# Kaixhin/Rainbow

Hardware: NVIDIA B200
Metric: learner updates/sec (batch32, 1M buffer, 51 atoms) (higher is better)
Workload: dtype f32

## Files before the change

### include/rainbow_b200.h

```cpp
#ifndef RAINBOW_B200_H
#define RAINBOW_B200_H

#include <stdint.h>

#ifdef __cplusplus
extern "C" {
#endif

#define RB_ABI_VERSION 2

#define RB_OK 0
#define RB_ERR_INVAL (-22)
#define RB_ERR_RANGE (-34)
#define RB_ERR_CUDA (-5)

#define RB_FRAME_BYTES 7056
#define RB_MAX_WINDOW 64
#define RB_MAX_ATOMS 128
#define RB_MAX_NOISY_LAYERS 8
#define RB_MAX_PEERS 8
#define RB_APPEND_BATCH 8


typedef void* rb_stream_t;

enum {
  RB_K_TREE_UPDATE = 0, RB_K_TREE_FIND, RB_K_TREE_SAMPLE, RB_K_GATHER, RB_K_ITER_STATES, RB_K_APPEND, RB_K_C51,
  RB_K_NOISY_RESAMPLE, RB_K_NOISY_COMPOSE, RB_K_SQNORM, RB_K_CLIP_ADAM, RB_K_HEAD_FC1, RB_K_HEAD_FC2, RB_K_HEAD_LOGITS,
  RB_K_HEAD_WGRAD2, RB_K_HEAD_DH, RB_K_HEAD_BWD1, RB_K_NOISE_FACTORS, RB_K_C51_DUELING, RB_K_BIAS_GRAD, RB_K_Q_VALUES,
  RB_K_HEAD_REDUCE1, RB_K_CONV_WGRAD, RB_KERNEL_COUNT
};

int rb_abi_version(void);
const char* rb_last_error(void);

int rb_profile_enable(int on);
int rb_profile_collect(int kernel_id, double* total_ms, int* launches);

int rb_tree_update(float* tree, int64_t tree_start, int64_t size, const int64_t* tree_idx,
                   const float* raw_priority, float omega, int omega_is_applied, int B, float* running_max,
                   int32_t* status, const int32_t* gate, rb_stream_t stream);

int rb_tree_find(const float* tree, int64_t tree_start, int64_t size, const double* values, int B, float* probs,
                 int64_t* data_idx, int64_t* tree_idx, rb_stream_t stream);

int rb_tree_sample(const float* tree, int64_t tree_start, int64_t size, const int64_t* ring_state, int n,
                   int history, const double* u01, int u01_attempts, uint64_t seed, uint64_t* rng_counter, int B,
                   float beta, const float* beta_dev, int max_attempts, float* probs, int64_t* data_idx,
                   int64_t* tree_idx, float* weights, int32_t* status, rb_stream_t stream);

int rb_gather(const uint8_t* frames, const int32_t* timestep, const int32_t* action, const float* reward,
              const uint8_t* nonterminal, int64_t size, const int64_t* data_idx, int B, int history, int n,
              const float* gamma_pow, float* states, float* next_states, int64_t* actions, float* returns,
              float* nonterminals, rb_stream_t stream);

int rb_iter_states(const uint8_t* frames, const int32_t* timestep, int64_t size, int64_t first, int count,
                   int history, float* out, rb_stream_t stream);

int rb_append(float* tree, int64_t tree_start, int64_t size, uint8_t* frames, int32_t* timestep, int32_t* action,
              float* reward, uint8_t* nonterminal, int64_t* ring_state, float* running_max,
              const float* state_last_frame, int32_t action_value, float reward_value, int terminal,
              rb_stream_t stream);

int rb_append_batch(float* tree, int64_t tree_start, int64_t size, uint8_t* frames, int32_t* timestep, int32_t* action,
                    float* reward, uint8_t* nonterminal, int64_t* ring_state, float* running_max,
                    const float* const* last_frames, const int32_t* actions, const float* rewards, const int32_t* terminals,
                    int k, rb_stream_t stream);

int rb_c51_loss_grad(const float* q_online_s, const float* q_online_ns, const float* q_target_ns,
                     const int64_t* actions, const float* returns, const float* nonterminals,
                     const float* weights, const float* support, float vmin, float vmax, float delta_z,
                     float gamma_n, int B, int A, int Z, float* loss, float* grad_q_online_s, float* m_out,
                     int64_t* astar_out, rb_stream_t stream);

int rb_noisy_resample(float* const* weight_eps, float* const* bias_eps, const int* in_features,
                      const int* out_features, int n_layers, const float* x_in, const float* x_out, uint64_t seed,
                      uint64_t* rng_counter, rb_stream_t stream);

int rb_noisy_outer(float* const* weight_eps, float* const* bias_eps, const int* in_features, const int* out_features,
                   int n_layers, const float* f_in, const float* f_out, rb_stream_t stream);

int rb_noise_factors(float* f_in, int n_in, float* f_out, int n_out, const float* x_in, const float* x_out, uint64_t seed,
                     uint64_t* rng_counter, rb_stream_t stream);

typedef struct rb_head_params {
  const float* w1_mu[2];    const float* w1_sigma[2];
  const float* b1_mu[2];    const float* b1_sigma[2];
  const float* w2_mu[2];    const float* w2_sigma[2];
  const float* b2_mu[2];    const float* b2_sigma[2];
  const float* eps_in1[2];  const float* eps_out1[2];
  const float* eps_in2[2];  const float* eps_out2[2];
  int conv_features, hidden, atoms, actions;
} rb_head_params;

typedef struct rb_head_grads {
  float* w1_mu[2]; float* w1_sigma[2]; float* b1_mu[2]; float* b1_sigma[2];
  float* w2_mu[2]; float* w2_sigma[2]; float* b2_mu[2]; float* b2_sigma[2];
} rb_head_grads;

int rb_head_splits(int conv_features, int hidden, int* s1, int* s2);
int rb_head_ticket_count(void);
int rb_head_debug(int flags);

int rb_head_forward(const rb_head_params* p, const float* x_lo, int m_lo, const float* x_hi, int m_hi, float* part1, float* part2,
                    int32_t* tickets, float* h, float* z, rb_stream_t stream);

int rb_head_logits(const float* z, int M, int actions, int atoms, float* q, rb_stream_t stream);

#define RB_HEAD_BWD_WGRAD2 1
#define RB_HEAD_BWD_DH 2
#define RB_HEAD_BWD_LAYER1 4
#define RB_HEAD_BWD_ALL 7
int rb_head_backward(const rb_head_params* p, const rb_head_grads* g, const float* x, const float* h, const float* dz, int B,
                     float* dh_scratch, float* dx, int relu_mask_x, int parts, rb_stream_t stream);

int rb_q_values(const float* z, int M, int actions, int atoms, const float* support, float* q, int64_t* best_action,
                float* best_q, rb_stream_t stream);

int rb_bias_grad(const float* grad_out, int B, int C, int HW, float* out, rb_stream_t stream);

int rb_conv_wgrad_scratch_elems(int B, int IC, int IH, int OC, int K, int stride);
int rb_conv_wgrad(const float* grad_out, const float* input, int B, int IC, int IH, int IW, int OC, int K, int stride,
                  float* partials, float* out, float* bias_out, rb_stream_t stream);

int rb_c51_dueling_loss_grad(const float* z_online, const float* z_target, int actions_n, int atoms, const int64_t* actions,
                             const float* returns, const float* nonterminals, const float* weights, const float* support,
                             float vmin, float vmax, float delta_z, float gamma_n, int B, float* loss, float* dz, float* m_out,
                             int64_t* astar_out, rb_stream_t stream);

int rb_noisy_compose(const float* mu, const float* sigma, const float* eps, int64_t count, float* out,
                     rb_stream_t stream);

int rb_clip_adam_scratch_elems(void);
int rb_clip_adam(float* param, const float* grad, float* exp_avg, float* exp_avg_sq, int64_t P, float grad_scale,
                 float max_norm, float lr, float beta1, float beta2, float eps, int64_t* step_count,
                 double* partial_sums, float* norm_out, const int32_t* gate, rb_stream_t stream);

int rb_peer_scratch_bytes(void);
int rb_peer_reduce(const float* const* peer_grad, uint64_t* const* peer_flags, int world, int rank, int seg, int64_t seg_begin,
                   int64_t seg_len, float grad_scale, float* gred_part, const uint64_t* epoch, void* scratch,
                   rb_stream_t stream);
int rb_peer_adam_gather(float* const* peer_param, uint64_t* const* peer_flags, double* const* peer_norms, int world, int rank,
                        int n_seg, const int64_t* seg_begin, const int64_t* seg_len, const float* gred, float* exp_avg,
                        float* exp_avg_sq, float max_norm, float lr, float beta1, float beta2, float eps, int64_t* step_count,
                        uint64_t* epoch, void* scratch, float* norm_out, float* multicast_param, rb_stream_t stream);
int rb_peer_clip_adam(const float* const* peer_grad, float* const* peer_param, uint64_t* const* peer_flags,
                      double* const* peer_norms, int world, int rank, int64_t P, float* gred, float* exp_avg,
                      float* exp_avg_sq, float grad_scale, float max_norm, float lr, float beta1, float beta2, float eps,
                      int64_t* step_count, uint64_t* epoch, void* scratch, float* norm_out, rb_stream_t stream);

#ifdef __cplusplus
}
#endif
#endif
```

### rainbow_b200/_lib.py

```python
import ctypes as C
import os

from . import _build

_lib = None

_vp, _i64, _i32, _f32, _u64 = C.c_void_p, C.c_int64, C.c_int, C.c_float, C.c_uint64

class HeadParams(C.Structure):
    _fields_ = [(n, _vp * 2) for n in ("w1_mu", "w1_sigma", "b1_mu", "b1_sigma", "w2_mu", "w2_sigma", "b2_mu", "b2_sigma",
                                        "eps_in1", "eps_out1", "eps_in2", "eps_out2")] + \
               [(n, C.c_int) for n in ("conv_features", "hidden", "atoms", "actions")]


class HeadGrads(C.Structure):
    _fields_ = [(n, _vp * 2) for n in ("w1_mu", "w1_sigma", "b1_mu", "b1_sigma", "w2_mu", "w2_sigma", "b2_mu", "b2_sigma")]


_hp, _hg = C.POINTER(HeadParams), C.POINTER(HeadGrads)

SIGNATURES = {
    "rb_abi_version": (C.c_int, []),
    "rb_last_error": (C.c_char_p, []),
    "rb_profile_enable": (C.c_int, [_i32]),
    "rb_profile_collect": (C.c_int, [_i32, C.POINTER(C.c_double), C.POINTER(C.c_int)]),
    "rb_tree_update": (C.c_int, [_vp, _i64, _i64, _vp, _vp, _f32, _i32, _i32, _vp, _vp, _vp, _vp]),
    "rb_tree_find": (C.c_int, [_vp, _i64, _i64, _vp, _i32, _vp, _vp, _vp, _vp]),
    "rb_tree_sample": (C.c_int, [_vp, _i64, _i64, _vp, _i32, _i32, _vp, _i32, _u64, _vp, _i32, _f32, _vp, _i32,
                                 _vp, _vp, _vp, _vp, _vp, _vp]),
    "rb_gather": (C.c_int, [_vp, _vp, _vp, _vp, _vp, _i64, _vp, _i32, _i32, _i32, _vp, _vp, _vp, _vp, _vp, _vp, _vp]),
    "rb_iter_states": (C.c_int, [_vp, _vp, _i64, _i64, _i32, _i32, _vp, _vp]),
    "rb_append": (C.c_int, [_vp, _i64, _i64, _vp, _vp, _vp, _vp, _vp, _vp, _vp, _vp, C.c_int32, _f32, _i32, _vp]),
    "rb_append_batch": (C.c_int, [_vp, _i64, _i64, _vp, _vp, _vp, _vp, _vp, _vp, _vp, _vp, _vp, _vp, _vp, _i32, _vp]),
    "rb_c51_loss_grad": (C.c_int, [_vp, _vp, _vp, _vp, _vp, _vp, _vp, _vp, _f32, _f32, _f32, _f32, _i32, _i32, _i32,
                                   _vp, _vp, _vp, _vp, _vp]),
    "rb_noisy_resample": (C.c_int, [_vp, _vp, _vp, _vp, _i32, _vp, _vp, _u64, _vp, _vp]),
    "rb_noisy_outer": (C.c_int, [_vp, _vp, _vp, _vp, _i32, _vp, _vp, _vp]),
    "rb_noise_factors": (C.c_int, [_vp, _i32, _vp, _i32, _vp, _vp, _u64, _vp, _vp]),
    "rb_head_splits": (C.c_int, [_i32, _i32, C.POINTER(C.c_int), C.POINTER(C.c_int)]),
    "rb_head_ticket_count": (C.c_int, []),
    "rb_head_debug": (C.c_int, [_i32]),
    "rb_head_forward": (C.c_int, [_hp, _vp, _i32, _vp, _i32, _vp, _vp, _vp, _vp, _vp, _vp]),
    "rb_head_logits": (C.c_int, [_vp, _i32, _i32, _i32, _vp, _vp]),
    "rb_head_backward": (C.c_int, [_hp, _hg, _vp, _vp, _vp, _i32, _vp, _vp, _i32, _i32, _vp]),
    "rb_bias_grad": (C.c_int, [_vp, _i32, _i32, _i32, _vp, _vp]),
    "rb_conv_wgrad_scratch_elems": (C.c_int, [_i32, _i32, _i32, _i32, _i32, _i32]),
    "rb_conv_wgrad": (C.c_int, [_vp, _vp, _i32, _i32, _i32, _i32, _i32, _i32, _i32, _vp, _vp, _vp, _vp]),
    "rb_c51_dueling_loss_grad": (C.c_int, [_vp, _vp, _i32, _i32, _vp, _vp, _vp, _vp, _vp, _f32, _f32, _f32, _f32, _i32,
                                           _vp, _vp, _vp, _vp, _vp]),
    "rb_noisy_compose": (C.c_int, [_vp, _vp, _vp, _i64, _vp, _vp]),
    "rb_peer_scratch_bytes": (C.c_int, []),
    "rb_peer_reduce": (C.c_int, [_vp, _vp, _i32, _i32, _i32, _i64, _i64, _f32, _vp, _vp, _vp, _vp]),
    "rb_peer_adam_gather": (C.c_int, [_vp, _vp, _vp, _i32, _i32, _i32, _vp, _vp, _vp, _vp, _vp, _f32, _f32, _f32, _f32, _f32,
                                      _vp, _vp, _vp, _vp, _vp, _vp]),
    "rb_peer_clip_adam": (C.c_int, [_vp, _vp, _vp, _vp, _i32, _i32, _i64, _vp, _vp, _vp, _f32, _f32, _f32, _f32, _f32, _f32,
                                    _vp, _vp, _vp, _vp, _vp]),
    "rb_clip_adam_scratch_elems": (C.c_int, []),
    "rb_clip_adam": (C.c_int, [_vp, _vp, _vp, _vp, _i64, _f32, _f32, _f32, _f32, _f32, _f32, _vp, _vp, _vp, _vp, _vp]),
    "rb_q_values": (C.c_int, [_vp, _i32, _i32, _i32, _vp, _vp, _vp, _vp, _vp]),
}


class RainbowB200Error(RuntimeError):
    pass


def load():
    global _lib
    if _lib is not None:
        return _lib
    if _build.stale():
        try:
            _build.build()
        except Exception as e:
            if not os.path.exists(_build.SO):
                raise RainbowB200Error(f"librainbow_b200.so is missing and could not be built: {e}") from e
    lib = C.CDLL(_build.SO)
    for name, (res, args) in SIGNATURES.items():
        fn = getattr(lib, name)
        fn.restype = res
        fn.argtypes = args
    if lib.rb_abi_version() != 2:
        raise RainbowB200Error("librainbow_b200.so ABI version mismatch")
    _lib = lib
    return lib


def check(rc):
    if rc != 0:
        raise RainbowB200Error(f"rainbow_b200 C ABI error {rc}: {load().rb_last_error().decode()}")


def ptr(t):
    if t is None:
        return None
    if not t.is_cuda:
        raise RainbowB200Error("rainbow_b200 kernels need CUDA tensors (no CPU fallback exists)")
    if not t.is_contiguous():
        raise RainbowB200Error("rainbow_b200 kernels need contiguous tensors")
    return t.data_ptr()


def stream():
    import torch
    return torch.cuda.current_stream().cuda_stream


KERNEL_IDS = ["tree_update", "tree_find", "tree_sample", "gather", "iter_states", "append", "c51", "noisy_resample",
              "noisy_compose", "sqnorm", "clip_adam", "head_fc1", "head_fc2", "head_logits", "head_wgrad2", "head_dh",
              "head_bwd1", "noise_factors", "c51_dueling", "bias_grad", "q_values", "head_reduce1", "conv_wgrad"]


class KernelTimer:

    def __enter__(self):
        check(load().rb_profile_enable(1))
        return self

    def __exit__(self, *exc):
        lib = load()
        check(lib.rb_profile_enable(0))
        self.result = {}
        for i, name in enumerate(KERNEL_IDS):
            ms, n = C.c_double(0.0), C.c_int(0)
            check(lib.rb_profile_collect(i, C.byref(ms), C.byref(n)))
            if n.value:
                self.result[name] = (n.value, 1e3 * ms.value / n.value)
        return False
```

### rainbow_b200/csrc/rb_head.cu

```cuda

#include <cooperative_groups.h>
#include <cuda_runtime.h>
#include <math_constants.h>
#include <stdint.h>
#include <stdio.h>

#include "rainbow_b200.h"
#include "rb_internal.cuh"

namespace cg = cooperative_groups;

namespace {

constexpr int HT = 128;
constexpr int NT = 64;
constexpr int KT = 32;
constexpr int LDB = NT + 4;
constexpr int FC_T = 256;

struct HeadDesc {
  const float* w1_mu[2]; const float* w1_sig[2]; const float* b1_mu[2]; const float* b1_sig[2];
  const float* w2_mu[2]; const float* w2_sig[2]; const float* b2_mu[2]; const float* b2_sig[2];
  const float* ei1[2]; const float* eo1[2]; const float* ei2[2]; const float* eo2[2];
  int K1, H, Z, A;
// ... 774 lines not shown
      const float* src = in + ((size_t)(b * IC + ic) * IH + (size_t)y0 * S) * IW;
      for (int i = tid; i < have_rows * IW; i += nthr) xs[ic * xs_ld + i] = __ldg(src + i);
    }
    for (int oc = 0; oc < OC; ++oc) {
      const float* src = g + ((size_t)(b * OC + oc) * OH + y0) * OW;
      for (int i = tid; i < rows * OW; i += nthr) gs[oc * (RB * OW) + i] = __ldg(src + i);
    }
  }
  __syncthreads();
  float* dst = part + (size_t)(b * gridDim.x + band) * (size_t)(n_w + OC);
  const bool vec = (S % 4 == 0) && (IW % 4 == 0);
  const int krows = IC * KW;
  const int kr = tid % krows, og = tid / krows;
  const int ic = kr / KW, ky = kr % KW;
  float acc[CW_OCT][KW];
#pragma unroll
  for (int i = 0; i < CW_OCT; ++i)
#pragma unroll
    for (int j = 0; j < KW; ++j) acc[i][j] = 0.0f;
  if (og * CW_OCT < OC) {
    for (int yy = 0; yy < rows; ++yy) {
      const float* xrow = xs + ic * xs_ld + (yy * S + ky) * IW;
      const float* grow = gs + (og * CW_OCT) * (RB * OW) + yy * OW;
      for (int xx = 0; xx < OW; ++xx) {
        float xv[KW], gv[CW_OCT];
        if ((KW % 4 == 0) && vec) {
#pragma unroll
          for (int j = 0; j < KW; j += 4) {
            const float4 v = *reinterpret_cast<const float4*>(xrow + xx * S + j);
            xv[j] = v.x; xv[j + 1] = v.y; xv[j + 2] = v.z; xv[j + 3] = v.w;
          }
        } else {
#pragma unroll
          for (int j = 0; j < KW; ++j) xv[j] = xrow[xx * S + j];
        }
#pragma unroll
        for (int i = 0; i < CW_OCT; ++i) gv[i] = grow[i * (RB * OW) + xx];
#pragma unroll
        for (int i = 0; i < CW_OCT; ++i)
#pragma unroll
          for (int j = 0; j < KW; ++j) acc[i][j] = fmaf(gv[i], xv[j], acc[i][j]);
      }
    }
#pragma unroll
    for (int i = 0; i < CW_OCT; ++i) {
      const int oc = og * CW_OCT + i;
      if (oc < OC) {
#pragma unroll
        for (int j = 0; j < KW; ++j) dst[((size_t)(oc * IC + ic) * KW + ky) * KW + j] = acc[i][j];
      }
    }
  }
  for (int oc = tid; oc < OC; oc += nthr) {
    float bsum = 0.0f;
    for (int i = 0; i < rows * OW; ++i) bsum += gs[oc * (RB * OW) + i];
    dst[n_w + oc] = bsum;
  }
}

constexpr int CWR_J = 64;

__global__ void __launch_bounds__(4 * CWR_J)
k_conv_wgrad_reduce(const float* __restrict__ part, int n_part, int n_w, int n_b, float* __restrict__ out_w,
                    float* __restrict__ out_b) {
  __shared__ float s_q[4][CWR_J];
  const int jl = threadIdx.x % CWR_J, q = threadIdx.x / CWR_J, j = blockIdx.x * CWR_J + jl, n = n_w + n_b;
  const int per = (n_part + 3) / 4, p_lo = q * per, p_hi = min(n_part, p_lo + per);
  float acc = 0.0f;
  if (j < n) {
    for (int p0 = p_lo; p0 < p_hi; p0 += 32) {
      float v[32];
#pragma unroll
      for (int u = 0; u < 32; ++u) v[u] = (p0 + u < p_hi) ? __ldcg(part + (size_t)(p0 + u) * n + j) : 0.0f;
#pragma unroll
      for (int u = 0; u < 32; ++u) acc += v[u];
    }
  }
  s_q[q][jl] = acc;
  __syncthreads();
  if (q == 0 && j < n) {
    const float t = ((s_q[0][jl] + s_q[1][jl]) + s_q[2][jl]) + s_q[3][jl];
    if (j < n_w) out_w[j] = t;
    else if (out_b) out_b[j - n_w] = t;
  }
}

int head_check(const rb_head_params* p, const char* who) {
  if (!p) return rbi::fail(RB_ERR_INVAL, who);
  for (int s = 0; s < 2; ++s)
    if (!p->w1_mu[s] || !p->w1_sigma[s] || !p->b1_mu[s] || !p->b1_sigma[s] || !p->w2_mu[s] || !p->w2_sigma[s] ||
        !p->b2_mu[s] || !p->b2_sigma[s])
      return rbi::fail(RB_ERR_INVAL, who);
  const bool noisy = p->eps_in1[0] != nullptr;
  for (int s = 0; s < 2; ++s)
    if ((p->eps_in1[s] != nullptr) != noisy || (p->eps_out1[s] != nullptr) != noisy || (p->eps_in2[s] != nullptr) != noisy ||
        (p->eps_out2[s] != nullptr) != noisy)
      return rbi::fail(RB_ERR_INVAL, "rb_head: give all eight noise factor vectors or none");
  if (p->conv_features <= 0 || p->hidden <= 0 || p->atoms <= 1 || p->actions <= 0) return rbi::fail(RB_ERR_INVAL, who);
  for (int s = 0; s < 2; ++s) {
    const uintptr_t bits = (uintptr_t)p->w1_mu[s] | (uintptr_t)p->w1_sigma[s] | (uintptr_t)p->b1_mu[s] | (uintptr_t)p->b1_sigma[s] |
                           (uintptr_t)p->w2_mu[s] | (uintptr_t)p->w2_sigma[s] | (uintptr_t)p->eps_in1[s] |
                           (uintptr_t)p->eps_out1[s] | (uintptr_t)p->eps_in2[s];
    if (bits & 15) return rbi::fail(RB_ERR_INVAL, "rb_head: weight / bias / factor pointers must be 16-byte aligned");
  }
  if (p->conv_features % 32 || p->hidden % 64) return rbi::fail(RB_ERR_RANGE, "rb_head: conv_features % 32 == 0 and hidden % 64 == 0 required");
  return RB_OK;
}

void head_splits(int K1, int H, int* s1, int* s2, int* ks1, int* ks2) {
  const int ntiles1 = 2 * H / NT;
  int want = (296 + ntiles1 - 1) / ntiles1;
  const int kt1 = (K1 + KT - 1) / KT;
  if (want > kt1) want = kt1;
  if (want > 16) want = 16;
  if (want < 1) want = 1;
  int per = (kt1 + want - 1) / want;
  *ks1 = per * KT;
  *s1 = (kt1 + per - 1) / per;
  const int kt2 = H / KT;
  int w2 = kt2 < 4 ? kt2 : 4;
  int per2 = (kt2 + w2 - 1) / w2;
  *ks2 = per2 * KT;
  *s2 = (kt2 + per2 - 1) / per2;
}

}

extern "C" {

int rb_head_splits(int conv_features, int hidden, int* s1, int* s2) {
  if (!s1 || !s2 || conv_features <= 0 || hidden <= 0) return rbi::fail(RB_ERR_INVAL, "rb_head_splits: bad argument");
  int a, b;
  head_splits(conv_features, hidden, s1, s2, &a, &b);
  int s_tc, per;
  rbi::head_fc1_tc_splits(conv_features, hidden, &s_tc, &per);
  if (s_tc > *s1) *s1 = s_tc;
  return RB_OK;
}

int rb_head_ticket_count(void) { return 4096; }

static int g_head_debug = 0;
int rb_head_debug(int flags) {
  g_head_debug = flags;
  return RB_OK;
}

int rb_head_forward(const rb_head_params* p, const float* x_lo, int m_lo, const float* x_hi, int m_hi, float* part1, float* part2,
                    int32_t* tickets, float* h, float* z, rb_stream_t stream) {
  int rc = head_check(p, "rb_head_forward: null pointer or bad size");
  if (rc != RB_OK) return rc;
  const int M = m_lo + m_hi;
  if (!x_lo || m_lo <= 0 || m_hi < 0 || (m_hi > 0 && !x_hi) || !part1 || !part2 || !tickets || !h || !z)
    return rbi::fail(RB_ERR_INVAL, "rb_head_forward: bad argument");
  const HeadDesc d = to_desc(p);
  int s1, s2, ks1, ks2;
  head_splits(d.K1, d.H, &s1, &s2, &ks1, &ks2);
  cudaStream_t st = (cudaStream_t)stream;
  const int MT = (M > 32) ? 64 : 32;
  const int mt = (M + MT - 1) / MT;
  const int tiles1 = 2 * d.H / NT, tiles2 = (d.Z + NT - 1) / NT + (d.A * d.Z + NT - 1) / NT;
  if (mt > 65535 || mt * tiles1 > 2048 || mt * tiles2 > 2048) return rbi::fail(RB_ERR_RANGE, "rb_head_forward: too many rows");
  const size_t smem64 = (size_t)FC_STAGES * (64 + 2 * NT) * (KT + 4) * sizeof(float);
  const size_t smem32 = (size_t)FC_STAGES * (32 + 2 * NT) * (KT + 4) * sizeof(float);
  rc = rbi::ensure_dynamic_smem(k_head_fc<64, 1>, smem64, "rb_head_forward");
  if (rc == RB_OK) rc = rbi::ensure_dynamic_smem(k_head_fc<64, 2>, smem64, "rb_head_forward");
// ... 54 lines not shown
    g.w1_mu[s] = gr->w1_mu[s]; g.w1_sig[s] = gr->w1_sigma[s]; g.b1_mu[s] = gr->b1_mu[s]; g.b1_sig[s] = gr->b1_sigma[s];
    g.w2_mu[s] = gr->w2_mu[s]; g.w2_sig[s] = gr->w2_sigma[s]; g.b2_mu[s] = gr->b2_mu[s]; g.b2_sig[s] = gr->b2_sigma[s];
  }
  const HeadDesc d = to_desc(p);
  cudaStream_t st = (cudaStream_t)stream;
  if (parts & RB_HEAD_BWD_WGRAD2) {
    const int tiles = (d.Z + NT - 1) / NT + (d.A * d.Z + NT - 1) / NT;
    dim3 grid(tiles, d.H / NT);
    rbi::ProfScope prof_(RB_K_HEAD_WGRAD2, st);
    k_head_wgrad2<<<grid, HT, 0, st>>>(d, g, dz, h, B);
  }
  rc = rbi::check_launch("rb_head_backward(wgrad2)");
  if (rc != RB_OK) return rc;
  if (parts & RB_HEAD_BWD_DH) {
    const int ns_max = d.A * d.Z > d.Z ? d.A * d.Z : d.Z;
    const int ld_dz = ns_max | 1;
    const size_t smem = ((size_t)32 * ld_dz + 2 * (size_t)((ns_max + 3) & ~3) * DH_KB) * sizeof(float);
    if (smem > 200 * 1024 || d.H % DH_KB) return rbi::fail(RB_ERR_RANGE, "rb_head_backward: actions * atoms too large for the dh kernel");
    rc = rbi::ensure_dynamic_smem(k_head_dh, smem, "rb_head_backward");
    if (rc != RB_OK) return rc;
    dim3 grid(d.H / DH_KB, 2);
    rbi::ProfScope prof_(RB_K_HEAD_DH, st);
    k_head_dh<<<grid, DH_T, smem, st>>>(d, dz, h, B, dh_scratch, dh_scratch + (size_t)B * 2 * d.H, ld_dz);
  }
  rc = rbi::check_launch("rb_head_backward(dh)");
  if (rc != RB_OK) return rc;
  if (parts & RB_HEAD_BWD_LAYER1) {
    if (d.H > 1024) return rbi::fail(RB_ERR_RANGE, "rb_head_backward: hidden <= 1024 required");
    dim3 grid(d.K1 / B1_K, 4);
    rbi::ProfScope prof_(RB_K_HEAD_BWD1, st);
    const size_t smem_b1 = (size_t)B1_STAGES * B1_STAGE * sizeof(float);
    rc = rbi::ensure_dynamic_smem(k_head_bwd1, smem_b1, "rb_head_backward");
    if (rc != RB_OK) return rc;
    k_head_bwd1<<<grid, B1_T, smem_b1, st>>>(d, g, x, dh_scratch, dh_scratch + (size_t)B * 2 * d.H, B, dx, relu_mask_x);
  }
  return rbi::check_launch("rb_head_backward(bwd1)");
}

int rb_bias_grad(const float* grad_out, int B, int C, int HW, float* out, rb_stream_t stream) {
  if (!grad_out || !out || B <= 0 || C <= 0 || HW <= 0) return rbi::fail(RB_ERR_INVAL, "rb_bias_grad: bad argument");
  {
    rbi::ProfScope prof_(RB_K_BIAS_GRAD, (cudaStream_t)stream);
    k_bias_grad<<<C, 256, 0, (cudaStream_t)stream>>>(grad_out, B, C, HW, out);
  }
  return rbi::check_launch("rb_bias_grad");
}

static int conv_wgrad_band_rows(int OH) { return OH >= 16 ? (OH + 7) / 8 : OH; }

int rb_conv_wgrad_scratch_elems(int B, int IC, int IH, int OC, int K, int stride) {
  if (B <= 0 || IC <= 0 || OC <= 0 || K <= 0 || stride <= 0 || IH < K) return 0;
  const int OH = (IH - K) / stride + 1, RB = conv_wgrad_band_rows(OH), bands = (OH + RB - 1) / RB;
  return B * bands * (OC * IC * K * K + OC);
}

int rb_conv_wgrad(const float* grad_out, const float* input, int B, int IC, int IH, int IW, int OC, int K, int stride,
                  float* partials, float* out, float* bias_out, rb_stream_t stream) {
  if (!grad_out || !input || !partials || !out) return rbi::fail(RB_ERR_INVAL, "rb_conv_wgrad: null pointer");
  if (B <= 0 || IC <= 0 || OC <= 0 || stride <= 0 || IH < K || IW < K) return rbi::fail(RB_ERR_INVAL, "rb_conv_wgrad: bad shape");
  if (K != 8 && K != 5 && K != 4 && K != 3) return rbi::fail(RB_ERR_RANGE, "rb_conv_wgrad: kernel sizes 3, 4, 5 and 8 are instantiated");
  const int OH = (IH - K) / stride + 1, OW = (IW - K) / stride + 1;
  const int RB = conv_wgrad_band_rows(OH), bands = (OH + RB - 1) / RB;
  const int threads = IC * K * ((OC + CW_OCT - 1) / CW_OCT);
  if (threads > 256 || B > 65535) return rbi::fail(RB_ERR_RANGE, "rb_conv_wgrad: IC * K * ceil(OC / 4) must not exceed 256 threads");
  const size_t smem = ((size_t)IC * ((RB - 1) * stride + K) * IW + (size_t)OC * RB * OW) * sizeof(float);
  if (smem > 200 * 1024) return rbi::fail(RB_ERR_RANGE, "rb_conv_wgrad: slab does not fit in shared memory");
  cudaStream_t st = (cudaStream_t)stream;
  dim3 grid(bands, B);
  int rc = RB_OK;
  {
    rbi::ProfScope prof_(RB_K_CONV_WGRAD, st);
#define RB_CW_LAUNCH(KW_)                                                                                              \
  rc = rbi::ensure_dynamic_smem(k_conv_wgrad_first<KW_>, smem, "rb_conv_wgrad");                                       \
  if (rc == RB_OK) k_conv_wgrad_first<KW_><<<grid, threads, smem, st>>>(grad_out, input, IC, IH, IW, OC, OH, OW, stride, RB, partials);
    if (K == 8) { RB_CW_LAUNCH(8) } else if (K == 5) { RB_CW_LAUNCH(5) } else if (K == 4) { RB_CW_LAUNCH(4) } else { RB_CW_LAUNCH(3) }
#undef RB_CW_LAUNCH
    if (rc != RB_OK) return rc;
    const int n_w = OC * IC * K * K;
    k_conv_wgrad_reduce<<<(n_w + OC + CWR_J - 1) / CWR_J, 4 * CWR_J, 0, st>>>(partials, B * bands, n_w, OC, out, bias_out);
  }
  return rbi::check_launch("rb_conv_wgrad");
}

int rb_noise_factors(float* f_in, int n_in, float* f_out, int n_out, const float* x_in, const float* x_out, uint64_t seed,
                     uint64_t* rng_counter, rb_stream_t stream) {
  if (!f_in || !f_out || n_in <= 0 || n_out <= 0) return rbi::fail(RB_ERR_INVAL, "rb_noise_factors: bad argument");
  if ((x_in == nullptr) != (x_out == nullptr)) return rbi::fail(RB_ERR_INVAL, "rb_noise_factors: give both x_in and x_out or neither");
  if (!x_in && !rng_counter) return rbi::fail(RB_ERR_INVAL, "rb_noise_factors: need injected normals or rng_counter");
  {
    rbi::ProfScope prof_(RB_K_NOISE_FACTORS, (cudaStream_t)stream);
    k_noise_factors<<<1, 1024, 0, (cudaStream_t)stream>>>(f_in, n_in, f_out, n_out, x_in, x_out, seed, (unsigned long long*)rng_counter);
  }
  return rbi::check_launch("rb_noise_factors");
}

}
```

### rainbow_b200/model.py

```python
import ctypes as C
import math

import torch
from torch import nn
from torch.nn import functional as F

from . import _lib

_ARCH = {
    "canonical": (((32, 8, 4), (64, 4, 2), (64, 3, 1)), 3136),
    "data-efficient": (((32, 5, 5), (64, 5, 5)), 576),
}


class NoisyLinear(nn.Module):

    def __init__(self, in_features, out_features, std_init=0.5):
        super().__init__()
        self.in_features, self.out_features, self.std_init = in_features, out_features, std_init
        self.weight_mu = nn.Parameter(torch.empty(out_features, in_features))
        self.weight_sigma = nn.Parameter(torch.empty(out_features, in_features))
        self.register_buffer("weight_epsilon", torch.zeros(out_features, in_features))
        self.bias_mu = nn.Parameter(torch.empty(out_features))
        self.bias_sigma = nn.Parameter(torch.empty(out_features))
        self.register_buffer("bias_epsilon", torch.zeros(out_features))
        self.reset_parameters()
        self._construction_noise()

    def _construction_noise(self):
        with torch.no_grad():
            x_in, x_out = torch.randn(self.in_features), torch.randn(self.out_features)
            self._f_in, self._f_out = x_in.sign() * x_in.abs().sqrt(), x_out.sign() * x_out.abs().sqrt()
            self.weight_epsilon.copy_(torch.outer(self._f_out, self._f_in))
            self.bias_epsilon.copy_(self._f_out)

    def reset_parameters(self):
        bound = 1.0 / math.sqrt(self.in_features)
        with torch.no_grad():
            self.weight_mu.uniform_(-bound, bound)
            self.bias_mu.uniform_(-bound, bound)
            self.weight_sigma.fill_(self.std_init / math.sqrt(self.in_features))
            self.bias_sigma.fill_(self.std_init / math.sqrt(self.out_features))

    def forward(self, x):
        if self.training:
            w = torch.addcmul(self.weight_mu, self.weight_sigma, self.weight_epsilon)
            b = torch.addcmul(self.bias_mu, self.bias_sigma, self.bias_epsilon)
            return F.linear(x, w, b)
        return F.linear(x, self.weight_mu, self.bias_mu)


def _layer_arrays(layers):
    n = len(layers)
    return ((C.c_void_p * n)(*[_lib.ptr(m.weight_epsilon) for m in layers]),
            (C.c_void_p * n)(*[_lib.ptr(m.bias_epsilon) for m in layers]),
            (C.c_int * n)(*[m.in_features for m in layers]), (C.c_int * n)(*[m.out_features for m in layers]), n)


def resample_noise(layers, seed, rng_counter, x_in=None, x_out=None):
    w, b, fin, fout, n = _layer_arrays(layers)
    _lib.check(_lib.load().rb_noisy_resample(w, b, fin, fout, n, _lib.ptr(x_in), _lib.ptr(x_out), seed,
                                             _lib.ptr(rng_counter), _lib.stream()))


class FusedHead:

    MAX_ROWS = 4096

    def __init__(self, net):
        self.net = net
        self.lib = _lib.load()
        s1, s2 = C.c_int(), C.c_int()
        _lib.check(self.lib.rb_head_splits(net.conv_output_size, net.hidden_size, C.byref(s1), C.byref(s2)))
        self.s1, self.s2 = s1.value, s2.value
        self.ncols = net.atoms * (1 + net.action_space)
        self._scratch = {}
        self._tickets = None

    @staticmethod
    def supported(net):
        return (net.conv_output_size % 32 == 0 and net.hidden_size % 64 == 0 and net.atoms <= 128 and
                next(net.parameters()).is_cuda)

    def params(self, noisy=None):
        net = self.net
        noisy = net.training if noisy is None else noisy
        p = _lib.HeadParams()
        (hv, ha), (zv, za) = (net.fc_h_v, net.fc_h_a), (net.fc_z_v, net.fc_z_a)
        for s, (l1, l2) in enumerate(((hv, zv), (ha, za))):
            p.w1_mu[s], p.w1_sigma[s] = _lib.ptr(l1.weight_mu), _lib.ptr(l1.weight_sigma)
# ... 95 lines not shown
        out, oi, oo = {}, 0, 0
        for name, m in self.named_children():
            if "fc" in name:
                out[name] = (self._f_in[oi:oi + m.in_features], self._f_out[oo:oo + m.out_features])
                oi, oo = oi + m.in_features, oo + m.out_features
        return out

    def reset_noise(self, x_in=None, x_out=None):
        if not self._f_in.is_cuda:
            raise _lib.RainbowB200Error("DQN.reset_noise needs the network on a CUDA device (no CPU fallback)")
        if x_in is None and self._noise_queue:
            x_in, x_out = self._noise_queue.pop(0)
        if x_in is None and self.lazy_noise and not torch.cuda.is_current_stream_capturing():
            self._noise_pending = True
            return
        self._noise_pending = False
        _lib.check(_lib.load().rb_noise_factors(_lib.ptr(self._f_in), self._f_in.numel(), _lib.ptr(self._f_out),
                                                self._f_out.numel(), _lib.ptr(x_in), _lib.ptr(x_out), self.noise_seed,
                                                _lib.ptr(self._noise_counter), _lib.stream()))
        self._eps_stale = True

    def flush_noise(self):
        if self._noise_pending:
            self._noise_pending = False
            lazy, self.lazy_noise = self.lazy_noise, False
            try:
                self.reset_noise()
            finally:
                self.lazy_noise = lazy

    def queue_noise(self, x_in, x_out):
        self._noise_queue.append((x_in.contiguous(), x_out.contiguous()))

    def materialise_noise(self):
        self.flush_noise()
        if self._eps_stale:
            w, b, fin, fout, n = _layer_arrays(self.noisy_layers())
            _lib.check(_lib.load().rb_noisy_outer(w, b, fin, fout, n, _lib.ptr(self._f_in), _lib.ptr(self._f_out),
                                                  _lib.stream()))
            self._eps_stale = False

    def _factors_from_buffers(self):
        with torch.no_grad():
            fi, fo = [], []
            for m in self.noisy_layers():
                b = m.bias_epsilon
                o = int(b.abs().argmax())
                fo.append(b.clone())
                fi.append(m.weight_epsilon[o] / b[o] if float(b[o]) != 0.0 else torch.zeros_like(m.weight_epsilon[0]))
            self._f_in.copy_(torch.cat(fi))
            self._f_out.copy_(torch.cat(fo))
        self._eps_stale = False

    def state_dict(self, *args, **kwargs):
        if self._f_in.is_cuda:
            self.flush_noise()
        if self._eps_stale and self._f_in.is_cuda:
            self.materialise_noise()
        return super().state_dict(*args, **kwargs)

    def load_state_dict(self, state_dict, *args, **kwargs):
        out = super().load_state_dict(state_dict, *args, **kwargs)
        self._noise_pending = False
        self._factors_from_buffers()
        return out

    def head(self):
        if self._head is None:
            self._head = FusedHead(self)
        return self._head

    def fused_ok(self, rows):
        return self.use_fused_head and rows <= FusedHead.MAX_ROWS and FusedHead.supported(self)

    def features(self, x):
        return self.convs(x).view(-1, self.conv_output_size)

    def conv_layers(self):
        return [m for m in self.convs if isinstance(m, nn.Conv2d)]

    def manual_conv_ok(self, x):
        return x.is_cuda and torch.backends.cudnn.enabled

    def conv_forward_saving(self, x):
        acts = [x]
        for m in self.conv_layers():
            acts.append(torch.cudnn_convolution_relu(acts[-1], m.weight, m.bias, m.stride, m.padding, m.dilation, m.groups))
        return acts

    def _own_wgrad_ok(self, m, a_in):
        k, s = m.kernel_size, m.stride
        return (self.use_own_wgrad and k[0] == k[1] and s[0] == s[1] and k[0] in (3, 4, 5, 8) and tuple(m.padding) == (0, 0) and
                tuple(m.dilation) == (1, 1) and m.groups == 1 and a_in.is_contiguous() and m.weight.grad.is_contiguous() and
                m.in_channels * k[0] * ((m.out_channels + 3) // 4) <= 256 and
                _lib.load().rb_conv_wgrad_scratch_elems(a_in.shape[0], m.in_channels, a_in.shape[2], m.out_channels, k[0], s[0]) > 0)

    def _wgrad_scratch(self, m, a_in):
        n = _lib.load().rb_conv_wgrad_scratch_elems(a_in.shape[0], m.in_channels, a_in.shape[2], m.out_channels, m.kernel_size[0], m.stride[0])
        buf = getattr(self, "_wgrad_buf", None)
        if buf is None or buf.numel() < n or buf.device != a_in.device:
            buf = torch.empty(n, dtype=torch.float32, device=a_in.device)
            self._wgrad_buf = buf
        return buf

    def conv_backward_into_grads(self, acts, g_last, side_stream, first_layer_stream=None):
        lib = _lib.load()
        main = torch.cuda.current_stream(g_last.device)
        layers = self.conv_layers()
        g = g_last
        extra_done = None
        for li in range(len(layers) - 1, -1, -1):
            m, a_in = layers[li], acts[li]
            ready = torch.cuda.Event()
            ready.record(main)
            own = li == 0 and self._own_wgrad_ok(m, a_in)
            st = first_layer_stream if (own and first_layer_stream is not None) else side_stream
            with torch.cuda.stream(st):
                st.wait_event(ready)
                g.record_stream(st)
                if own:
                    _lib.check(lib.rb_conv_wgrad(_lib.ptr(g), _lib.ptr(a_in), a_in.shape[0], a_in.shape[1], a_in.shape[2], a_in.shape[3],
                                                 m.out_channels, m.kernel_size[0], m.stride[0], _lib.ptr(self._wgrad_scratch(m, a_in)),
                                                 _lib.ptr(m.weight.grad), _lib.ptr(m.bias.grad), st.cuda_stream))
                else:
                    _lib.check(lib.rb_bias_grad(_lib.ptr(g), g.shape[0], g.shape[1], g.shape[2] * g.shape[3],
                                                _lib.ptr(m.bias.grad), st.cuda_stream))
                    _, gw, _ = torch.ops.aten.convolution_backward(g, a_in, m.weight, None, m.stride, m.padding, m.dilation, False,
                                                                   [0, 0], m.groups, [False, True, False])
                    m.weight.grad.copy_(gw)
                if st is not side_stream:
                    extra_done = torch.cuda.Event()
                    extra_done.record(st)
            if li > 0:
                gin, _, _ = torch.ops.aten.convolution_backward(g, a_in, m.weight, None, m.stride, m.padding, m.dilation, False,
                                                                [0, 0], m.groups, [True, False, False])
                g = torch.ops.aten.threshold_backward(gin, a_in, 0.0)
        if extra_done is not None:
            side_stream.wait_event(extra_done)
        done = torch.cuda.Event()
        done.record(side_stream)
        return done

    def features_nograd(self, x):
        if not (x.is_cuda and torch.backends.cudnn.enabled):
            return self.features(x)
        for m in self.convs:
            if isinstance(m, nn.Conv2d):
                x = torch.cudnn_convolution_relu(x, m.weight, m.bias, m.stride, m.padding, m.dilation, m.groups)
        return x.view(-1, self.conv_output_size)

    def logits(self, x):
        feats = self.features(x)
        recording = torch.is_grad_enabled() and (feats.requires_grad or self.fc_h_v.weight_mu.requires_grad)
        if not recording and self.fused_ok(feats.shape[0]):
            z, _, _ = self.head().forward(feats.contiguous())
            return self.head().logits(z)
        if self._eps_stale:
            self.materialise_noise()
        v = self.fc_z_v(F.relu(self.fc_h_v(feats))).view(-1, 1, self.atoms)
        a = self.fc_z_a(F.relu(self.fc_h_a(feats))).view(-1, self.action_space, self.atoms)
        return v + a - a.mean(1, keepdim=True)

    def forward(self, x, log=False):
        q = self.logits(x)
        return F.log_softmax(q, dim=2) if log else F.softmax(q, dim=2)
```

Before: 3077.

## Add custom implicit-GEMM conv forward kernel using 3xTF32 tensor-core MMA

Replaces the cuDNN fused conv+ReLU forward with a hand-written implicit-GEMM kernel. Each block stages an input row band and 32 output-channel weight rows in shared memory and runs split-precision (3x) TF32 mma for near-FP32 accuracy. A split-K reduction goes through shared memory, and bias plus ReLU are fused at the end. The aim is to cut cuDNN dispatch overhead and poor utilisation at batch 32. The risk is that a hand-tuned kernel may be slower than cuDNN, and the 3x MMA adds compute.

```diff
diff --git a/include/rainbow_b200.h b/include/rainbow_b200.h
--- a/include/rainbow_b200.h
+++ b/include/rainbow_b200.h
@@ -28,7 +28,7 @@
   RB_K_TREE_UPDATE = 0, RB_K_TREE_FIND, RB_K_TREE_SAMPLE, RB_K_GATHER, RB_K_ITER_STATES, RB_K_APPEND, RB_K_C51,
   RB_K_NOISY_RESAMPLE, RB_K_NOISY_COMPOSE, RB_K_SQNORM, RB_K_CLIP_ADAM, RB_K_HEAD_FC1, RB_K_HEAD_FC2, RB_K_HEAD_LOGITS,
   RB_K_HEAD_WGRAD2, RB_K_HEAD_DH, RB_K_HEAD_BWD1, RB_K_NOISE_FACTORS, RB_K_C51_DUELING, RB_K_BIAS_GRAD, RB_K_Q_VALUES,
-  RB_K_HEAD_REDUCE1, RB_K_CONV_WGRAD, RB_KERNEL_COUNT
+  RB_K_HEAD_REDUCE1, RB_K_CONV_WGRAD, RB_K_CONV_FWD, RB_KERNEL_COUNT
 };
 
 int rb_abi_version(void);
@@ -123,6 +123,9 @@
 int rb_conv_wgrad(const float* grad_out, const float* input, int B, int IC, int IH, int IW, int OC, int K, int stride,
                   float* partials, float* out, float* bias_out, rb_stream_t stream);
 
+int rb_conv_forward(const float* input, const float* weight, const float* bias, int B, int IC, int IH, int IW, int OC, int K,
+                    int stride, float* out, rb_stream_t stream);
+
 int rb_c51_dueling_loss_grad(const float* z_online, const float* z_target, int actions_n, int atoms, const int64_t* actions,
                              const float* returns, const float* nonterminals, const float* weights, const float* support,
                              float vmin, float vmax, float delta_z, float gamma_n, int B, float* loss, float* dz, float* m_out,
diff --git a/rainbow_b200/_lib.py b/rainbow_b200/_lib.py
--- a/rainbow_b200/_lib.py
+++ b/rainbow_b200/_lib.py
@@ -46,6 +46,7 @@
     "rb_bias_grad": (C.c_int, [_vp, _i32, _i32, _i32, _vp, _vp]),
     "rb_conv_wgrad_scratch_elems": (C.c_int, [_i32, _i32, _i32, _i32, _i32, _i32]),
     "rb_conv_wgrad": (C.c_int, [_vp, _vp, _i32, _i32, _i32, _i32, _i32, _i32, _i32, _vp, _vp, _vp, _vp]),
+    "rb_conv_forward": (C.c_int, [_vp, _vp, _vp, _i32, _i32, _i32, _i32, _i32, _i32, _i32, _vp, _vp]),
     "rb_c51_dueling_loss_grad": (C.c_int, [_vp, _vp, _i32, _i32, _vp, _vp, _vp, _vp, _vp, _f32, _f32, _f32, _f32, _i32,
                                            _vp, _vp, _vp, _vp, _vp]),
     "rb_noisy_compose": (C.c_int, [_vp, _vp, _vp, _i64, _vp, _vp]),
@@ -108,7 +109,7 @@
 
 KERNEL_IDS = ["tree_update", "tree_find", "tree_sample", "gather", "iter_states", "append", "c51", "noisy_resample",
               "noisy_compose", "sqnorm", "clip_adam", "head_fc1", "head_fc2", "head_logits", "head_wgrad2", "head_dh",
-              "head_bwd1", "noise_factors", "c51_dueling", "bias_grad", "q_values", "head_reduce1", "conv_wgrad"]
+              "head_bwd1", "noise_factors", "c51_dueling", "bias_grad", "q_values", "head_reduce1", "conv_wgrad", "conv_fwd"]
 
 
 class KernelTimer:
diff --git a/rainbow_b200/csrc/rb_head.cu b/rainbow_b200/csrc/rb_head.cu
--- a/rainbow_b200/csrc/rb_head.cu
+++ b/rainbow_b200/csrc/rb_head.cu
@@ -880,6 +880,164 @@
     const float t = ((s_q[0][jl] + s_q[1][jl]) + s_q[2][jl]) + s_q[3][jl];
     if (j < n_w) out_w[j] = t;
     else if (out_b) out_b[j - n_w] = t;
+  }
+}
+
+__device__ __forceinline__ void tf32_split_rn(float v, uint32_t& hi, uint32_t& lo) {
+  asm("cvt.rna.tf32.f32 %0, %1;" : "=r"(hi) : "f"(v));
+  lo = __float_as_uint(__fsub_rn(v, __uint_as_float(hi)));
+}
+
+constexpr int CF_T = 256;
+constexpr int CF_WARPS = CF_T / 32;
+constexpr int CF_OC = 32;
+constexpr int CF_MAX_BAND = 5;
+
+struct ConvFwdCfg {
+  int OH, OW, RB, bands, in_rows, npx, groups, ksplit, kdim, kpad, nk, ldw, ldr, slab;
+  size_t smem;
+};
+
+ConvFwdCfg conv_fwd_cfg(int IC, int IH, int IW, int K, int S) {
+  ConvFwdCfg c;
+  c.OH = (IH - K) / S + 1;
+  c.OW = (IW - K) / S + 1;
+  const int nb = (c.OH + CF_MAX_BAND - 1) / CF_MAX_BAND;
+  c.RB = (c.OH + nb - 1) / nb;
+  c.bands = (c.OH + c.RB - 1) / c.RB;
+  c.in_rows = (c.RB - 1) * S + K;
+  c.npx = c.RB * c.OW;
+  c.groups = ((c.npx + 7) / 8 + 1) / 2;
+  c.kdim = IC * K * K;
+  c.kpad = (c.kdim + 7) & ~7;
+  c.nk = c.kpad / 8;
+  c.ksplit = CF_WARPS / c.groups;
+  if (c.ksplit < 1) c.ksplit = 1;
+  if (c.ksplit > c.nk) c.ksplit = c.nk;
+  c.ldw = ((c.kpad + 31) & ~31) + 4;
+  c.ldr = c.groups * 16 + 4;
+  c.slab = (IC * c.in_rows * IW + 3) & ~3;
+  c.smem = ((size_t)c.slab + (size_t)CF_OC * c.ldw + (size_t)c.ksplit * CF_OC * c.ldr + (size_t)c.kpad) * sizeof(float);
+  return c;
+}
+
+template <int K, int S>
+__global__ void __launch_bounds__(CF_T)
+k_conv_fwd(const float* __restrict__ x, const float* __restrict__ w, const float* __restrict__ bias, int IC, int IH, int IW,
+           int OC, const ConvFwdCfg c, float* __restrict__ y) {
+  extern __shared__ __align__(16) float cf_smem[];
+  float* xs = cf_smem;
+  float* ws = xs + c.slab;
+  float* red = ws + (size_t)CF_OC * c.ldw;
+  int* koff = reinterpret_cast<int*>(red + (size_t)c.ksplit * CF_OC * c.ldr);
+  const int tid = threadIdx.x, band = blockIdx.x, oc0 = blockIdx.y * CF_OC, b = blockIdx.z;
+  const int y0 = band * c.RB, rows = min(c.RB, c.OH - y0), npx = rows * c.OW;
+  const int have_rows = min(c.in_rows, IH - y0 * S);
+  const int xs_ld = c.in_rows * IW;
+
+  const float* xsrc = x + ((size_t)b * IC * IH + (size_t)y0 * S) * IW;
+  const int chunk = have_rows * IW;
+  if ((IW & 3) == 0 && ((uintptr_t)x & 15) == 0) {
+    const int q = chunk >> 2;
+    for (int i = tid; i < IC * q; i += CF_T) {
+      const int ic = i / q, j = i - ic * q;
+      cp_async16(xs + ic * xs_ld + 4 * j, xsrc + (size_t)ic * IH * IW + 4 * j);
+    }
+  } else {
+    for (int i = tid; i < IC * chunk; i += CF_T) {
+      const int ic = i / chunk, j = i - ic * chunk;
+      cp_async4(xs + ic * xs_ld + j, xsrc + (size_t)ic * IH * IW + j);
+    }
+  }
+  const float* wsrc = w + (size_t)oc0 * c.kdim;
+  if ((c.kdim & 3) == 0 && ((uintptr_t)w & 15) == 0) {
+    const int q = c.kdim >> 2;
+    for (int i = tid; i < CF_OC * q; i += CF_T) {
+      const int r = i / q, j = i - r * q;
+      cp_async16(ws + r * c.ldw + 4 * j, wsrc + (size_t)r * c.kdim + 4 * j);
+    }
+  } else {
+    for (int i = tid; i < CF_OC * c.kdim; i += CF_T) {
+      const int r = i / c.kdim, j = i - r * c.kdim;
+      cp_async4(ws + r * c.ldw + j, wsrc + (size_t)r * c.kdim + j);
+    }
+  }
+  for (int i = tid; i < CF_OC * (c.kpad - c.kdim); i += CF_T) {
+    const int r = i / (c.kpad - c.kdim), j = c.kdim + i % (c.kpad - c.kdim);
+    ws[r * c.ldw + j] = 0.0f;
+  }
+  for (int k = tid; k < c.kpad; k += CF_T) {
+    const int ic = k / (K * K), r = k - ic * (K * K), ky = r / K, kx = r - ky * K;
+    koff[k] = (k < c.kdim) ? ic * xs_ld + ky * IW + kx : 0;
+  }
+  cp_async_wait_all();
+  __syncthreads();
+
+  const int warp = tid >> 5, lane = tid & 31, gid = lane >> 2, tig = lane & 3;
+  const int units = c.groups * c.ksplit, per = (c.nk + c.ksplit - 1) / c.ksplit;
+  for (int u = warp; u < units; u += CF_WARPS) {
+    const int grp = u % c.groups, ks = u / c.groups;
+    float acc[2][2][4];
+#pragma unroll
+    for (int i = 0; i < 2; ++i)
+#pragma unroll
+      for (int j = 0; j < 2; ++j)
+#pragma unroll
+        for (int q = 0; q < 4; ++q) acc[i][j][q] = 0.0f;
+    int poff[2];
+#pragma unroll
+    for (int j = 0; j < 2; ++j) {
+      const int p = grp * 16 + 8 * j + gid;
+      const int oy = p / c.OW, ox = p - oy * c.OW;
+      poff[j] = (p < npx) ? oy * S * IW + ox * S : 0;
+    }
+    const int s_begin = ks * per, s_end = min(c.nk, s_begin + per);
+    for (int s = s_begin; s < s_end; ++s) {
+      const int k0 = 8 * s;
+      uint32_t ahi[2][4], alo[2][4];
+#pragma unroll
+      for (int i = 0; i < 2; ++i) {
+        const float* a = ws + (16 * i) * c.ldw + k0;
+        tf32_split_rn(a[gid * c.ldw + tig], ahi[i][0], alo[i][0]);
+        tf32_split_rn(a[(gid + 8) * c.ldw + tig], ahi[i][1], alo[i][1]);
+        tf32_split_rn(a[gid * c.ldw + tig + 4], ahi[i][2], alo[i][2]);
+        tf32_split_rn(a[(gid + 8) * c.ldw + tig + 4], ahi[i][3], alo[i][3]);
+      }
+      const int ko0 = koff[k0 + tig], ko1 = koff[k0 + tig + 4];
+#pragma unroll
+      for (int j = 0; j < 2; ++j) {
+        uint32_t bhi[2], blo[2];
+        tf32_split_rn(xs[ko0 + poff[j]], bhi[0], blo[0]);
+        tf32_split_rn(xs[ko1 + poff[j]], bhi[1], blo[1]);
+#pragma unroll
+        for (int i = 0; i < 2; ++i) {
+          float d[4] = {0.0f, 0.0f, 0.0f, 0.0f};
+          mma_tf32(d, alo[i], bhi);
+          mma_tf32(d, ahi[i], blo);
+          mma_tf32(d, ahi[i], bhi);
+#pragma unroll
+          for (int q = 0; q < 4; ++q) acc[i][j][q] += d[q];
+        }
+      }
+    }
+    float* dst = red + (size_t)ks * CF_OC * c.ldr + grp * 16;
+#pragma unroll
+    for (int i = 0; i < 2; ++i)
+#pragma unroll
+      for (int j = 0; j < 2; ++j)
+#pragma unroll
+        for (int h = 0; h < 2; ++h)
+          *reinterpret_cast<float2*>(dst + (16 * i + gid + 8 * h) * c.ldr + 8 * j + 2 * tig) =
+              make_float2(acc[i][j][2 * h], acc[i][j][2 * h + 1]);
+  }
+  __syncthreads();
+  const size_t ohw = (size_t)c.OH * c.OW;
+  float* yb = y + ((size_t)b * OC + oc0) * ohw + (size_t)y0 * c.OW;
+  for (int i = tid; i < CF_OC * npx; i += CF_T) {
+    const int oc = i / npx, p = i - oc * npx;
+    float v = red[oc * c.ldr + p];
+    for (int ks = 1; ks < c.ksplit; ++ks) v += red[((size_t)ks * CF_OC + oc) * c.ldr + p];
+    yb[(size_t)oc * ohw + p] = fmaxf(v + __ldg(bias + oc0 + oc), 0.0f);
   }
 }
 
@@ -1100,6 +1258,31 @@
   return rbi::check_launch("rb_conv_wgrad");
 }
 
+int rb_conv_forward(const float* input, const float* weight, const float* bias, int B, int IC, int IH, int IW, int OC, int K,
+                    int stride, float* out, rb_stream_t stream) {
+  if (!input || !weight || !bias || !out) return rbi::fail(RB_ERR_INVAL, "rb_conv_forward: null pointer");
+  if (B <= 0 || IC <= 0 || OC <= 0 || K <= 0 || stride <= 0 || IH < K || IW < K) return rbi::fail(RB_ERR_INVAL, "rb_conv_forward: bad shape");
+  const bool inst = (K == 8 && stride == 4) || (K == 4 && stride == 2) || (K == 3 && stride == 1) || (K == 5 && stride == 5);
+  if (!inst) return rbi::fail(RB_ERR_RANGE, "rb_conv_forward: (kernel, stride) in {(8,4), (4,2), (3,1), (5,5)} are instantiated");
+  if (OC % CF_OC) return rbi::fail(RB_ERR_RANGE, "rb_conv_forward: out_channels % 32 == 0 required");
+  const ConvFwdCfg c = conv_fwd_cfg(IC, IH, IW, K, stride);
+  if (c.smem > 200 * 1024) return rbi::fail(RB_ERR_RANGE, "rb_conv_forward: input band and weight rows do not fit in shared memory");
+  if (B > 65535) return rbi::fail(RB_ERR_RANGE, "rb_conv_forward: at most 65535 rows");
+  cudaStream_t st = (cudaStream_t)stream;
+  dim3 grid(c.bands, OC / CF_OC, B);
+  int rc = RB_OK;
+  {
+    rbi::ProfScope prof_(RB_K_CONV_FWD, st);
+#define RB_CF_LAUNCH(K_, S_)                                                                                           \
+  rc = rbi::ensure_dynamic_smem(k_conv_fwd<K_, S_>, c.smem, "rb_conv_forward");                                       \
+  if (rc == RB_OK) k_conv_fwd<K_, S_><<<grid, CF_T, c.smem, st>>>(input, weight, bias, IC, IH, IW, OC, c, out);
+    if (K == 8) { RB_CF_LAUNCH(8, 4) } else if (K == 4) { RB_CF_LAUNCH(4, 2) } else if (K == 3) { RB_CF_LAUNCH(3, 1) } else { RB_CF_LAUNCH(5, 5) }
+#undef RB_CF_LAUNCH
+  }
+  if (rc != RB_OK) return rc;
+  return rbi::check_launch("rb_conv_forward");
+}
+
 int rb_noise_factors(float* f_in, int n_in, float* f_out, int n_out, const float* x_in, const float* x_out, uint64_t seed,
                      uint64_t* rng_counter, rb_stream_t stream) {
   if (!f_in || !f_out || n_in <= 0 || n_out <= 0) return rbi::fail(RB_ERR_INVAL, "rb_noise_factors: bad argument");
diff --git a/rainbow_b200/model.py b/rainbow_b200/model.py
--- a/rainbow_b200/model.py
+++ b/rainbow_b200/model.py
@@ -6,6 +6,8 @@
 from torch.nn import functional as F
 
 from . import _lib
+
+RB_ERR_RANGE = -34
 
 _ARCH = {
     "canonical": (((32, 8, 4), (64, 4, 2), (64, 3, 1)), 3136),
@@ -267,10 +269,33 @@
     def manual_conv_ok(self, x):
         return x.is_cuda and torch.backends.cudnn.enabled
 
-    def conv_forward_saving(self, x):
+    def _own_conv_body(self, x):
+        if not (x.is_cuda and x.dtype == torch.float32 and x.is_contiguous() and x.dim() == 4):
+            return None
+        lib = _lib.load()
         acts = [x]
         for m in self.conv_layers():
-            acts.append(torch.cudnn_convolution_relu(acts[-1], m.weight, m.bias, m.stride, m.padding, m.dilation, m.groups))
+            a = acts[-1]
+            if (m.padding != (0, 0) or m.dilation != (1, 1) or m.groups != 1 or m.kernel_size[0] != m.kernel_size[1] or
+                    m.stride[0] != m.stride[1] or not (m.weight.is_contiguous() and m.bias.is_contiguous())):
+                return None
+            k, s = m.kernel_size[0], m.stride[0]
+            y = torch.empty((a.shape[0], m.out_channels, (a.shape[2] - k) // s + 1, (a.shape[3] - k) // s + 1),
+                            dtype=torch.float32, device=a.device)
+            rc = lib.rb_conv_forward(_lib.ptr(a), _lib.ptr(m.weight), _lib.ptr(m.bias), a.shape[0], a.shape[1], a.shape[2], a.shape[3],
+                                     m.out_channels, k, s, _lib.ptr(y), _lib.stream())
+            if rc == RB_ERR_RANGE:
+                return None
+            _lib.check(rc)
+            acts.append(y)
+        return acts
+
+    def conv_forward_saving(self, x):
+        acts = self._own_conv_body(x)
+        if acts is None:
+            acts = [x]
+            for i in range(0, len(self.convs), 2):
+                acts.append(self.convs[i + 1](self.convs[i](acts[-1])))
         return acts
 
     def _own_wgrad_ok(self, m, a_in):
@@ -327,12 +352,10 @@
         return done
 
     def features_nograd(self, x):
-        if not (x.is_cuda and torch.backends.cudnn.enabled):
+        acts = self._own_conv_body(x)
+        if acts is None:
             return self.features(x)
-        for m in self.convs:
-            if isinstance(m, nn.Conv2d):
-                x = torch.cudnn_convolution_relu(x, m.weight, m.bias, m.stride, m.padding, m.dilation, m.groups)
-        return x.view(-1, self.conv_output_size)
+        return acts[-1].view(-1, self.conv_output_size)
 
     def logits(self, x):
         feats = self.features(x)
```

New measurement: 3316 (median of 6 runs). 1.08x the previous value.
